# plumer/pbrs

Hardware: AMD Instinct MI355X
Metric: Msamples/s (higher is better)
Workload: dtype f32

## Files before the change

### pbrs_amd/csrc/device/scene.h

```cpp
#pragma once
#include <stddef.h>
#include <stdint.h>

#include "../../../include/pbrs_gpu.h"

constexpr uint32_t kBlock = 256;
constexpr size_t kLdsBytesPerCU = 160 * 1024;

struct pbrs_wnode;
struct DevScene {
    const pbrs_node* nodes;
    const pbrs_instance* inst;
    const pbrs_shape* shapes;
    const pbrs_mesh* meshes;
    const pbrs_tri_verts* tv;
    const pbrs_tri_shade* ts;
    const pbrs_material* mats;
    const pbrs_bxdf* bxdfs;
    const pbrs_area_light* alights;
    const pbrs_delta_light* dlights;
    uint32_t n_area, n_delta;
    float env[3];
    uint32_t has_env;
    uint32_t fast_slab;
    uint32_t exact_extent;
    uint32_t flat_off, n_flat;
    uint32_t features;
    uint32_t refill_below;
    uint32_t refill_below_shadow;
    const pbrs_texture* textures;
    const float* tex_floats;
    const uint32_t* tex_words;
    uint32_t env_kind, env_texture;
    float env_scale[3];
    const pbrs_fourier_table* fourier;
    uint32_t n_classes;
    const pbrs_wnode* wnodes;
    uint32_t wide_cap;
    uint32_t lds_off_words, lds_nodes, lds_tris, lds_inst, lds_shapes;
    const pbrs_node* nodes_top;
    uint32_t n_inst, n_shapes, n_tris, n_mats, n_bxdfs;
};

#define PBRS_INSTANCE_TRANSLATION 0x100u
#define PBRS_FEAT_ANALYTIC 1u
#define PBRS_FEAT_SHADING_CHECK 2u
#define PBRS_FEAT_FLAT_TLAS 4u
#define PBRS_FEAT_ALL 7u
#define PBRS_FEAT_EXTENT 256u
#define PBRS_FEAT_LONG_WALKS 8u
#define PBRS_FEAT_WIDE 16u
#define PBRS_FEAT_LDS_TOP 128u
#define PBRS_FEAT_LDS_SCENE 64u
#define PBRS_FEAT_FULL_STEPS 32u
#define PBRS_FLAT_TLAS_MIN 2u
#ifndef PBRS_FLAT_TLAS_MAX
#define PBRS_FLAT_TLAS_MAX 20u
#endif
#ifndef PBRS_FLAT_TLAS_MAX_ANYHIT
#define PBRS_FLAT_TLAS_MAX_ANYHIT 32u
#endif

struct pbrs_wnode {
    float lo[3][4];
    float hi[3][4];
    uint32_t child[4];
    uint32_t pad[4];
};
#ifndef PBRS_WIDE_STACK_MAX
#define PBRS_WIDE_STACK_MAX 16
#endif
#ifndef PBRS_WIDE_MIN_LEVELS
#define PBRS_WIDE_MIN_LEVELS 4u
#endif
#define PBRS_WREF_LEAF 0x80000000u
#define PBRS_WREF_NONE 0xffffffffu
#define PBRS_WREF_INDEX 0x07ffffffu
#define PBRS_WREF_AXIS_SHIFT 27
#define PBRS_WIDE_UNUSED_PLANE 1152921504606846976.0f

#ifndef PBRS_REFILL_BELOW_SHORT
#define PBRS_REFILL_BELOW_SHORT 20u
#endif
#ifndef PBRS_REFILL_BELOW_LONG
#define PBRS_REFILL_BELOW_LONG 48u
#endif
#ifndef PBRS_REFILL_BELOW_LONG_SHADOW
#define PBRS_REFILL_BELOW_LONG_SHADOW 40u
#endif
#define PBRS_LONG_WALK_HEIGHT 12u

#define PBRS_SHADE_LAMBERT 1u
#define PBRS_SHADE_LIGHT_SPHERE 2u
#define PBRS_SHADE_LIGHT_TRIANGLE 4u
#define PBRS_SHADE_FOURIER 8u
#define PBRS_SHADE_FOURIER_ONLY 16u
#define PBRS_SHADE_LDS_RECORDS 32u
#define PBRS_SHADE_LDS_TRIS 64u
#define PBRS_MAX_CLASSES 16u

#define PBRS_PERSISTENT_BLOCKS 1536
#ifndef PBRS_WORK_HEADS
#define PBRS_WORK_HEADS 8u
#endif
#define PBRS_WORK_HEAD_STRIDE 32u
#define PBRS_SORT_TILE 16384u
#define PBRS_QSPLIT_ON 1u
#define PBRS_QSPLIT_ENV 2u
```

### pbrs_amd/csrc/device/shadow.h

```cpp
#pragma once
#include "extend.h"

template <bool STATS, uint32_t FEAT>
__global__ void __launch_bounds__(256, STATS ? 3 : (FEAT & PBRS_FEAT_WIDE) ? PBRS_WIDE_SHADOW_WAVES : PBRS_SHADOW_WAVES)
    k_shadow(DevScene G, PathState st, const uint32_t* count, uint32_t* next, GlobalCounters* gc, const uint32_t* indirect, uint32_t* slow_list,
             uint32_t* slow_count) {
    extern __shared__ __attribute__((aligned(16))) uint32_t lds_stack[];
    const DevScene S = (!STATS && (FEAT & PBRS_FEAT_LDS_SCENE)) ? stage_scene(G, lds_stack) : (!STATS && (FEAT & PBRS_FEAT_LDS_TOP)) ? stage_top(G, lds_stack) : G;
    constexpr uint32_t ARITY = PBRS_WALK_ARITY(STATS, FEAT);
    constexpr bool WIDE = ARITY != 0u;
    const uint32_t n = indirect ? count[0] : count[1];
    LaneStack stk{lds_stack + threadIdx.x, st.sr[0], st.sr[1], 0u};
    Cnt<STATS> cnt;
    cnt.init();
    uint32_t nrays = 0;
    typename AnySel<ARITY, STATS, (FEAT & (PBRS_FEAT_ALL | PBRS_FEAT_LDS_TOP))>::type walk;
    walk.mode = PBRS_WALK_IDLE;
    PBRS_KP_DECL(walk);
    PBRS_TT_DECL;
    uint32_t item = 0, rec = 0;
    f3 l_vis = gray(0.0f);
    WaveWork work = wave_work_init(n);
    for (;;) {
        uint64_t live = __ballot(walk.mode == PBRS_WALK_NODE || walk.mode == PBRS_WALK_LEAF || walk.mode == PBRS_WALK_XFER);
        if ((uint32_t)__popcll(live) < S.refill_below_shadow) {
            PBRS_KP_WAVE(1);
            if constexpr (WIDE) {
                wave_append_slow(walk.mode == PBRS_WALK_SLOW, rec, slow_list, slow_count);
                if (walk.mode == PBRS_WALK_SLOW) walk.mode = PBRS_WALK_IDLE;
            }
            if (walk.mode == PBRS_WALK_DONE) {
                const bool occluded = walk.occluded;
                const uint32_t slot = item & PBRS_SLOT_MASK, r = item >> 31;
                if (item & 0x40000000u) {
                    if (!occluded) {
                        float* l = reinterpret_cast<float*>(st.L + slot);
                        l[0] = l_vis.x;
                        l[1] = l_vis.y;
                        l[2] = l_vis.z;
                    }
                } else {
                    at(st.occ[r], slot) = occluded ? 1 : 0;
                }
                walk.mode = PBRS_WALK_IDLE;
            }
            if (work.left()) {
                uint32_t idx = wave_fetch(work, walk.mode == PBRS_WALK_IDLE, next, n);
                if (idx != 0xffffffffu) {
                    if (indirect) idx = indirect[idx];
                    rec = idx;
                    stk.item = idx;
                    const float4 q0 = st.sr[0][idx], q1 = st.sr[1][idx];
                    item = __float_as_uint(q1.w);
                    if (item & 0x40000000u) l_vis = xyz(st.sr[2][idx]);
                    walk.start(S, mk3(q0.x, q0.y, q0.z), mk3(q1.x, q1.y, q1.z), q0.w, stk);
                    nrays++;
                    PBRS_KP_LANE(2, true);
                }
                if constexpr (WIDE) walk.scan_wave(S, stk);
                else walk.scan_wave(S, cnt);
                live = __ballot(walk.mode == PBRS_WALK_NODE || walk.mode == PBRS_WALK_LEAF || walk.mode == PBRS_WALK_XFER);
            }
            if (live == 0) {
                if constexpr (WIDE) {
                    walk.forget_reciprocals();
                    if (__ballot(walk.mode == PBRS_WALK_SLOW || walk.mode == PBRS_WALK_DONE)) continue;
                }
                break;
            }
        }
        PBRS_TT(0);
        PBRS_STEP_WALK(walk, S, stk, cnt, PBRS_SHD_XFER_MIN, PBRS_SHD_LEAF_MIN, PBRS_WALK_NSTEPS(FEAT, ARITY), ((FEAT & PBRS_FEAT_FULL_STEPS) != 0u));
        if constexpr (WIDE) walk.forget_reciprocals();
    }
    flush_counters<STATS>(cnt, gc, true, nrays, 0u);
    if (!STATS) PBRS_KP_FLUSH(1, walk);
    if (!STATS) PBRS_TT_FLUSH(1);
}
```

### pbrs_amd/csrc/device/traverse.h

```cpp
#pragma once
#include "shapes.h"

#include "probes.h"

struct RaySpace {
    f3 o, d;
    f3 nr;
    bool fast;
};
PD uint32_t dir_in_range(float x) {
    uint32_t e = (pn_bits(x) >> 23) & 0xffu;
    return (e - (127u - 40u) <= 80u) ? 1u : 0u;
}
PD uint32_t origin_in_range(float x) {
    uint32_t u = pn_bits(x) & 0x7fffffffu;
    uint32_t e = u >> 23;
    return ((u == 0u) | (e - (127u - 60u) <= 100u)) ? 1u : 0u;
}
PD RaySpace make_space(f3 o, f3 d, bool scene_ok) {
    RaySpace r;
    r.o = o;
    r.d = d;
    r.fast = ((scene_ok ? 1u : 0u) & dir_in_range(d.x) & dir_in_range(d.y) & dir_in_range(d.z) & origin_in_range(o.x) &
              origin_in_range(o.y) & origin_in_range(o.z)) != 0u;
// ... 695 lines not shown
            if (space == PBRS_SPACE_TRANSLATED) inst_kind |= 0x100u;
            stk.put(sp++, H.blas_root);
        } else if (inst_kind == PBRS_SHAPE_TRIANGLE) {
            leaf_a = H.blas_root;
            leaf_end = H.blas_root + 1u;
            mode = PBRS_WALK_LEAF;
        }
    }
    template <class AfterLeaf>
    PD void share_leaf(const DevScene& S, Cnt<STATS>& cnt, AfterLeaf after_leaf) {
        const bool tri_leaf = mode == PBRS_WALK_LEAF;
        TriShare sh;
        sh.build(tri_leaf ? leaf_end - leaf_a : 0u);
        if (sh.has[0] == 0) return;
        const f3 ho = sh.from_owner(C.o), hd = sh.from_owner(C.d);
        const float htmax = sh.from_owner(t_max);
        const uint32_t hti = sh.from_owner(leaf_a) + sh.k();
        bool hit = false;
        if (sh.helper()) {
            PBRS_TP(5);
            pbrs_tri_verts tv = load_tri(S.tv + hti);
            hit = mesh_tri_pred(tv, ho, hd, htmax);
        }
        const uint64_t hits = __ballot(hit);
        if (tri_leaf) {
            uint32_t tested = sh.cnt;
            bool occ = false;
#pragma unroll
            for (uint32_t j = 4u; j-- > 0u;) {
                if (j < sh.cnt && ((hits >> sh.pos(j)) & 1ull)) {
                    tested = j + 1u;
                    occ = true;
                }
            }
            if (STATS) cnt.c.triangles += tested;
            leaf_a += sh.cnt;
            mode = leaf_a != leaf_end ? PBRS_WALK_LEAF : after_leaf();
            if (occ) {
                occluded = true;
                mode = PBRS_WALK_DONE;
            }
        }
    }
    PD void leaf_wave(const DevScene& S, Cnt<STATS>& cnt) {
        share_leaf(S, cnt, [&]() __attribute__((always_inline)) { return sp == blas_base ? PBRS_WALK_XFER : PBRS_WALK_NODE; });
    }
    PD void analytic_visit(const DevScene& S, const pbrs_instance& in, Cnt<STATS>& cnt) {
        bool hit;
        {
            if (!(FEAT & PBRS_FEAT_ANALYTIC)) return;
            const f3 o = xf_apply(in.inv, C.o, 1.0f), d = xf_apply(in.inv, C.d, 0.0f);
            const float* p = S.shapes[in.shape_index].p;
            switch (inst_kind) {
                case PBRS_SHAPE_SPHERE:
                    CNT(spheres);
                    hit = sphere_occludes(ld3(p), p[3], o, d, t_max);
                    break;
                case PBRS_SHAPE_QUAD:
                    CNT(quads);
                    hit = quad_occludes(ld3(p), ld3(p + 3), ld3(p + 6), o, d, t_max);
                    break;
                case PBRS_SHAPE_CUBOID:
                    CNT(cuboids);
                    hit = slab_test(ld3(p), ld3(p + 3), o, d, t_max);
                    break;
                case PBRS_SHAPE_DISK:
                    CNT(disks);
                    hit = disk_occludes(ld3(p), ld3(p + 3), ld3(p + 6), o, d);
                    break;
                default:
                    hit = false;
                    break;
            }
        }
        if (hit) {
            occluded = true;
            mode = PBRS_WALK_DONE;
        }
    }
};

#define PBRS_WALK_SLOW 6u
#define PBRS_LEAF_UNVERIFIED 0xffffffffu
template <uint32_t FEAT>
struct AnyWalkW : AnyWalk<false, FEAT> {
    using B = AnyWalk<false, FEAT>;
    using B::C; using B::t_max; using B::leaf_a; using B::leaf_end; using B::inst_kind; using B::sp; using B::blas_base; using B::cand; using B::in_blas;
    using B::occluded; using B::moved; using B::mode;
    WideRay W;
    uint32_t cur;
    PD RaySpace exact_w() const {
        RaySpace E = C;
        E.nr = -W.r32;
        return E;
    }

    PD void start(const DevScene& S, f3 o, f3 d, float tmax, LaneStack stk) {
        B::start(S, o, d, tmax, stk);
        cur = PBRS_WREF_NONE;
        W.set(C);
        if (mode != PBRS_WALK_SCAN) mode = PBRS_WALK_SLOW;
    }
    PD void scan_wave(const DevScene& S, LaneStack) {
        Cnt<false> cnt;
        B::scan_wave(S, cnt);
    }
    PD uint32_t after_leaf() const { return sp == 0 ? B::exit_mode() : PBRS_WALK_NODE; }
    PD void hold_leaf(uint32_t ref) {
        leaf_a = ref & PBRS_WREF_INDEX;
        leaf_end = PBRS_LEAF_UNVERIFIED;
        mode = PBRS_WALK_LEAF;
    }
    PD void forget_reciprocals() { C.nr = gray(0.0f); }
    PD void node_step_fast(const DevScene& S, LaneStack stk, Cnt<false>& cnt) {
        if (cur == PBRS_WREF_NONE && sp == 0) return;
        node_step(S, stk, cnt);
    }
    PD void node_step(const DevScene& S, LaneStack stk, Cnt<false>&) {
        PBRS_TP(0);
        uint32_t e = cur;
        if (e == PBRS_WREF_NONE) {
            if (!in_blas) {
                if (cand == 0u) {
                    mode = PBRS_WALK_DONE;
                    return;
                }
                leaf_a = (uint32_t)__builtin_ctz(cand);
                cand &= cand - 1u;
                mode = PBRS_WALK_XFER;
                return;
            }
            if (sp == 0) {
                mode = B::exit_mode();
                return;
            }
            e = stk.get(--sp);
        }
        cur = PBRS_WREF_NONE;
        if (e & PBRS_WREF_LEAF) {
            hold_leaf(e);
            return;
        }
        PBRS_TP(1);
        const WideTest t = wide_test(S.wnodes, e, C, W, t_max);
        if (t.pass == 0u) {
            PBRS_TP(2);
            if (sp == 0) mode = B::exit_mode();
            return;
        }
        if (sp + 3 > (int)S.wide_cap) {
            mode = PBRS_WALK_SLOW;
            return;
        }
        const uint32_t first = wide_push(wide_order_any(t, C.d), stk, sp);
        if (first & PBRS_WREF_LEAF) hold_leaf(first);
        else cur = first;
    }
    PD void xfer_step(const DevScene& S, LaneStack stk, Cnt<false>& cnt) {
        if (in_blas) {
            const bool rebuilt = moved && !(inst_kind & 0x100u);
            mode = PBRS_WALK_NODE;
            in_blas = false;
            leave_instance(S, stk, !moved ? PBRS_SPACE_WORLD : (inst_kind & 0x100u) ? PBRS_SPACE_TRANSLATED : PBRS_SPACE_MOVED, C);
            if (rebuilt) W.set(C);
            return;
        }
        mode = PBRS_WALK_NODE;
        PBRS_TP(6);
        const pbrs_node leaf = load_node(S.nodes + S.flat_off + leaf_a);
        leaf_a = leaf.a;
        inst_kind = (leaf.b >> PBRS_TLAS_LEAF_KIND_SHIFT) & 7u;
        const pbrs_instance& in = S.inst[leaf_a];
        if ((FEAT & PBRS_FEAT_ANALYTIC) && inst_kind != PBRS_SHAPE_MESH && inst_kind != PBRS_SHAPE_TRIANGLE) {
            B::analytic_visit(S, in, cnt);
            return;
        }
        const InstHead H = load_inst_head(in);
        const uint32_t space = enter_instance(S, in, H.flags, C, inst_kind == PBRS_SHAPE_MESH, stk);
        moved = space != PBRS_SPACE_WORLD;
        in_blas = true;
        blas_base = 0;
        if (inst_kind == PBRS_SHAPE_MESH) {
            if (!C.fast) {
                mode = PBRS_WALK_SLOW;
                return;
            }
            if (space == PBRS_SPACE_TRANSLATED) inst_kind |= 0x100u;
            if (space == PBRS_SPACE_MOVED) W.set(C);
            const uint32_t wroot = H.wide_root;
            if (wroot == PBRS_WREF_NONE) {
                hold_leaf(H.blas_root);
                return;
            }
            if (!slab_rs(load_node(S.nodes + H.blas_root), exact_w(), t_max)) {
                mode = B::exit_mode();
                return;
            }
            cur = wroot;
        } else if (inst_kind == PBRS_SHAPE_TRIANGLE) {
            leaf_a = H.blas_root;
            leaf_end = H.blas_root + 1u;
            mode = PBRS_WALK_LEAF;
        }
    }
    PD void leaf_wave(const DevScene& S, Cnt<false>& cnt) {
        if (mode == PBRS_WALK_LEAF && leaf_end == PBRS_LEAF_UNVERIFIED) {
            PBRS_TP(3);
            const pbrs_node node = load_node(S.nodes + leaf_a);
            leaf_a = node.a;
            leaf_end = slab_rs(node, exact_w(), t_max) ? node.a + (node.b & ~PBRS_LEAF_FLAG) : node.a;
            if (leaf_end != leaf_a) PBRS_TP(4);
            if (leaf_end == leaf_a) mode = after_leaf();
        }
        B::share_leaf(S, cnt, [&]() __attribute__((always_inline)) { return after_leaf(); });
    }
};

template <bool STATS, uint32_t EXTRA = 0u>
PD void tlas_closest(const DevScene& S, bool active, f3 o, f3 d, float t_max, LaneStack stk, Hit& best, Cnt<STATS>& cnt) {
    ClosestWalk<STATS, PBRS_FEAT_ALL | EXTRA> w;
    w.start(S, o, d, t_max, stk);
    if (!active) w.mode = PBRS_WALK_DONE;
    w.scan_wave(S, cnt);
    while (__ballot(w.mode != PBRS_WALK_DONE)) {
        if (w.mode == PBRS_WALK_XFER) w.xfer_step(S, stk, cnt);
        if (w.mode == PBRS_WALK_NODE) w.node_step(S, stk, cnt);
        if (__ballot(w.mode == PBRS_WALK_LEAF)) w.leaf_wave(S, cnt);
    }
    w.finish(cnt);
    best = w.best;
}
template <bool STATS>
PD bool tlas_any(const DevScene& S, bool active, f3 o, f3 d, float t_max, LaneStack stk, Cnt<STATS>& cnt) {
    AnyWalk<STATS, PBRS_FEAT_ALL> w;
    w.start(S, o, d, t_max, stk);
    if (!active) w.mode = PBRS_WALK_DONE;
    w.scan_wave(S, cnt);
    while (__ballot(w.mode != PBRS_WALK_DONE)) {
        if (w.mode == PBRS_WALK_XFER) w.xfer_step(S, stk, cnt);
        if (w.mode == PBRS_WALK_NODE) w.node_step(S, stk, cnt);
        if (__ballot(w.mode == PBRS_WALK_LEAF)) w.leaf_wave(S, cnt);
    }
    return w.occluded;
}
PD bool tlas_any_wide(const DevScene& S, bool active, f3 o, f3 d, float t_max, LaneStack stk, bool& slow) {
    Cnt<false> cnt;
    AnyWalkW<PBRS_FEAT_ALL> w;
    w.start(S, o, d, t_max, stk);
    if (!active) w.mode = PBRS_WALK_DONE;
    w.scan_wave(S, stk);
    while (__ballot(w.mode == PBRS_WALK_NODE || w.mode == PBRS_WALK_LEAF || w.mode == PBRS_WALK_XFER)) {
        if (w.mode == PBRS_WALK_XFER) w.xfer_step(S, stk, cnt);
        if (w.mode == PBRS_WALK_NODE) w.node_step(S, stk, cnt);
        if (__ballot(w.mode == PBRS_WALK_LEAF)) w.leaf_wave(S, cnt);
    }
    slow = w.mode == PBRS_WALK_SLOW;
    bool occ = w.occluded;
    if (__ballot(slow)) {
        const bool o2 = tlas_any<false>(S, active && slow, o, d, t_max, stk, cnt);
        if (slow) occ = o2;
    }
    return occ;
}
```

### pbrs_amd/csrc/device/wide.h

```cpp
#pragma once
#include "scene.h"
#include "shapes.h"


struct WideRay {
    f3 r32;
    uint32_t nb;
    PD void set(const RaySpace& C) {
        r32 = -C.nr;
        nb = (C.d.x > 0.0f ? 0u : 48u) | (C.d.y > 0.0f ? 16u : 64u) << 8 | (C.d.z > 0.0f ? 32u : 80u) << 16;
    }
    PD uint32_t nx() const { return nb & 0xffu; }
    PD uint32_t ny() const { return (nb >> 8) & 0xffu; }
    PD uint32_t nz() const { return nb >> 16; }
};

struct WideTest {
    uint32_t pass;
    uint32_t child[4];
    PD int axis_x() const { return (int)((child[0] >> PBRS_WREF_AXIS_SHIFT) & 3u); }
    PD int axis_left() const { return (int)((child[0] >> (PBRS_WREF_AXIS_SHIFT + 2)) & 3u); }
    PD int axis_right() const { return (int)((child[2] >> PBRS_WREF_AXIS_SHIFT) & 3u); }
};
PD WideTest wide_test(const pbrs_wnode* nodes, uint32_t wi, const RaySpace& C, const WideRay& W, float t_max) {
    const char* base = reinterpret_cast<const char*>(nodes);
    const uint32_t at = wi * (uint32_t)sizeof(pbrs_wnode);
    const float4 nx = *reinterpret_cast<const float4*>(base + (at + W.nx())), ny = *reinterpret_cast<const float4*>(base + (at + W.ny())),
                 nz = *reinterpret_cast<const float4*>(base + (at + W.nz()));
    const float4 fx = *reinterpret_cast<const float4*>(base + (at + (48u - W.nx()))), fy = *reinterpret_cast<const float4*>(base + (at + (80u - W.ny()))),
                 fz = *reinterpret_cast<const float4*>(base + (at + (112u - W.nz())));
    const uint4 ch = *reinterpret_cast<const uint4*>(base + (at + 96u));
    WideTest t;
    t.child[0] = ch.x, t.child[1] = ch.y, t.child[2] = ch.z, t.child[3] = ch.w;
    const uint32_t p0 = pn_slab_filter(nx.x, ny.x, nz.x, fx.x, fy.x, fz.x, C.o.x, C.o.y, C.o.z, W.r32.x, W.r32.y, W.r32.z, t_max) ? 1u : 0u;
    const uint32_t p1 = pn_slab_filter(nx.y, ny.y, nz.y, fx.y, fy.y, fz.y, C.o.x, C.o.y, C.o.z, W.r32.x, W.r32.y, W.r32.z, t_max) ? 2u : 0u;
    const uint32_t p2 = pn_slab_filter(nx.z, ny.z, nz.z, fx.z, fy.z, fz.z, C.o.x, C.o.y, C.o.z, W.r32.x, W.r32.y, W.r32.z, t_max) ? 4u : 0u;
    const uint32_t p3 = pn_slab_filter(nx.w, ny.w, nz.w, fx.w, fy.w, fz.w, C.o.x, C.o.y, C.o.z, W.r32.x, W.r32.y, W.r32.z, t_max) ? 8u : 0u;
    t.pass = p0 | p1 | p2 | p3;
    asm volatile("" : "+v"(t.child[0]), "+v"(t.child[1]), "+v"(t.child[2]), "+v"(t.child[3]));
    return t;
}

struct WideOrder {
    uint32_t r[4], p[4];
};
PD WideOrder wide_order_any(const WideTest& t, f3 d) {
    const bool sx = !(comp(d, t.axis_x()) > 0.0f);
    const uint32_t q0 = t.pass & 1u, q1 = (t.pass >> 1) & 1u, q2 = (t.pass >> 2) & 1u, q3 = (t.pass >> 3) & 1u;
    WideOrder o;
    o.r[0] = sx ? t.child[3] : t.child[0], o.r[1] = sx ? t.child[2] : t.child[1], o.r[2] = sx ? t.child[1] : t.child[2], o.r[3] = sx ? t.child[0] : t.child[3];
    o.p[0] = sx ? q3 : q0, o.p[1] = sx ? q2 : q1, o.p[2] = sx ? q1 : q2, o.p[3] = sx ? q0 : q3;
    return o;
}
PD uint32_t wide_push(const WideOrder& o, LaneStack stk, int& sp) {
    const uint32_t any01 = o.p[0] | o.p[1], any012 = any01 | o.p[2];
    if (o.p[3] & any012) stk.put(sp, o.r[3]);
    if (o.p[2] & any01) stk.put(sp + (int)o.p[3], o.r[2]);
    if (o.p[1] & o.p[0]) stk.put(sp + (int)(o.p[3] + o.p[2]), o.r[1]);
    sp += (int)(o.p[0] + o.p[1] + o.p[2] + o.p[3]) - 1;
    return o.p[0] ? o.r[0] : o.p[1] ? o.r[1] : o.p[2] ? o.r[2] : o.r[3];
}
```

### pbrs_amd/csrc/host/scene_prepare.cpp

```cpp
#include "scene_prepare.h"

#include <algorithm>
#include <cstring>
#include <map>
#include <string>

#include "../../../include/pbrs_numeric.h"
#include "../../../include/pbrs_scene_spec.h"
#include "../device/split_planes.h"

namespace pbrs {
namespace {

SceneCheck refuse(int code, const char* message) { return SceneCheck{code, message, SceneLevels{}}; }

void tree_heights(const pbrs_node* nodes, uint32_t n, std::vector<uint32_t>& h) {
    h.assign(n, 1u);
    for (uint32_t i = n; i-- > 0;)
        if (!(nodes[i].b & PBRS_LEAF_FLAG)) h[i] = std::max(h[i + 1], h[nodes[i].a]) + 1u;
}

SceneLevels scene_levels(const pbrs_scene_desc& d) {
    SceneLevels l;
    std::vector<uint32_t> th, bh;
// ... 177 lines not shown
    PreparedScene P;
    DevScene& S = P.S;
    SceneFacts& f = P.facts;
    P.stack_depth = lv.stack;
    {
        bool ok = true;
        for (uint32_t i = 0; i < d.n_tlas_nodes && ok; ++i)
            for (int a = 0; a < 3; ++a) ok = ok && coord_ok(d.tlas_nodes[i].min[a]) && coord_ok(d.tlas_nodes[i].max[a]);
        for (uint32_t i = 0; i < d.n_blas_nodes && ok; ++i)
            for (int a = 0; a < 3; ++a) ok = ok && coord_ok(d.blas_nodes[i].min[a]) && coord_ok(d.blas_nodes[i].max[a]);
        S.fast_slab = ok ? 1u : 0u;
    }
    S.exact_extent = lv.exact_extent ? 1u : 0u;

    const bool scan = tlas_scanned(d);
    std::vector<pbrs_node>& nodes = P.nodes;
    nodes.assign(d.tlas_nodes, d.tlas_nodes + d.n_tlas_nodes);
    S.flat_off = (uint32_t)nodes.size();
    if (scan)
        for (uint32_t i = 0; i < d.n_tlas_nodes; ++i)
            if (d.tlas_nodes[i].b & PBRS_LEAF_FLAG) nodes.push_back(d.tlas_nodes[i]);
    S.n_flat = (uint32_t)nodes.size() - S.flat_off;
    const uint64_t blas_off = nodes.size();
    nodes.insert(nodes.end(), d.blas_nodes, d.blas_nodes + d.n_blas_nodes);
    for (size_t i = blas_off; i < nodes.size(); ++i)
        if (!(nodes[i].b & PBRS_LEAF_FLAG)) nodes[i].a += (uint32_t)blas_off;
    P.node_planes.assign(nodes.size(), 0u);
    if (S.fast_slab != 0u)
        for (size_t i = blas_off; i < nodes.size(); ++i)
            if (!(nodes[i].b & PBRS_LEAF_FLAG)) P.node_planes[i] = split_planes(nodes, (uint32_t)i);
    P.walk_bytes = nodes.size() * sizeof(pbrs_node) + (uint64_t)d.n_triangles * sizeof(pbrs_tri_verts) + (uint64_t)d.n_instances * sizeof(pbrs_instance);

    std::vector<pbrs_instance>& inst = P.inst;
    inst.assign(d.instances, d.instances + d.n_instances);
    std::vector<uint32_t> mat_class(d.n_materials, 0u);
    {
        std::vector<std::string> sigs;
        for (uint32_t m = 0; m < d.n_materials; ++m) {
            const pbrs_material& mt = d.materials[m];
            if (mt.n_bxdfs == 0) continue;
            std::string sig;
            for (uint32_t k = 0; k < mt.n_bxdfs; ++k) {
                const pbrs_bxdf& bx = d.bxdfs[mt.first_bxdf + k];
                sig += (char)('a' + bx.kind);
                sig += (char)('a' + (bx.kind == PBRS_BXDF_SPECULAR ? bx.intrusion : 0u));
                sig += (char)('a' + (bx.kind == PBRS_BXDF_DIFFUSE ? bx.oren_nayar : bx.fresnel));
                sig += (char)('a' + (bx.kind == PBRS_BXDF_MICROFACET && bx.alpha_x != bx.alpha_y ? 1 : 0));
                sig += bx.tex ? 't' : '-';
            }
            size_t at = 0;
            while (at < sigs.size() && sigs[at] != sig) ++at;
            if (at == sigs.size()) sigs.push_back(sig);
            mat_class[m] = (uint32_t)std::min<size_t>(at + 1, PBRS_MAX_CLASSES - 1);
        }
        S.n_classes = (uint32_t)std::min<size_t>(sigs.size(), PBRS_MAX_CLASSES - 1);
        const std::string lam_sig = {(char)('a' + PBRS_BXDF_DIFFUSE), 'a', 'a', 'a', '-'};
        for (size_t at = 0; at < sigs.size() && at + 1 < PBRS_MAX_CLASSES - 1; ++at)
            if (sigs[at] == lam_sig) f.lambert_class = (uint32_t)at + 1;
        const std::string fou_sig = {(char)('a' + PBRS_BXDF_FOURIER), 'a', 'a', 'a', '-'};
        for (size_t at = 0; at < sigs.size() && at + 1 < PBRS_MAX_CLASSES - 1; ++at)
            if (sigs[at] == fou_sig) f.fourier_class = (uint32_t)at + 1;
    }
    for (pbrs_instance& in : inst) {
        in.pad[0] = mat_class[in.material];
        if (in.shape_kind == PBRS_SHAPE_MESH) in.blas_root += (uint32_t)blas_off;
        bool linear_identity = true;
        for (int r = 0; r < 3; ++r)
            for (int k = 0; k < 3; ++k) linear_identity = linear_identity && pn_bits(in.inv[r][k]) == pn_bits(r == k ? 1.0f : 0.0f);
        in.flags &= ~PBRS_INSTANCE_TRANSLATION;
        if (linear_identity) in.flags |= PBRS_INSTANCE_TRANSLATION;
    }
    for (pbrs_instance& in : inst) in.pad[1] = PBRS_WREF_NONE;
    S.wide_cap = 4u;
    if (scan && S.fast_slab != 0u) {
        std::vector<pbrs_wnode>& wide = P.wide;
        std::map<uint32_t, uint32_t> wide_of_root;
        uint32_t levels = 0;
        for (pbrs_instance& in : inst) {
            if (in.shape_kind != PBRS_SHAPE_MESH || (nodes[in.blas_root].b & PBRS_LEAF_FLAG)) continue;
            auto it = wide_of_root.find(in.blas_root);
            if (it == wide_of_root.end()) it = wide_of_root.emplace(in.blas_root, build_wide(nodes, in.blas_root, wide, 0u, levels)).first;
            in.pad[1] = it->second;
        }
        if (levels >= PBRS_WIDE_MIN_LEVELS && wide.size() * sizeof(pbrs_wnode) < (1ull << 32)) {
            P.walk_bytes += wide.size() * sizeof(pbrs_wnode);
            S.wide_cap = std::max(4u, std::min(3u * levels + 1u, (uint32_t)PBRS_WIDE_STACK_MAX));
            P.wide_levels = levels;
        } else {
            wide.clear();
            for (pbrs_instance& in : inst) in.pad[1] = PBRS_WREF_NONE;
        }
    }

    S.n_area = d.n_area_lights;
    S.n_delta = d.n_delta_lights;
    S.env_kind = d.env_kind;
    S.env_texture = d.env_texture;
    std::memcpy(S.env_scale, d.env_scale, sizeof S.env_scale);
    std::memcpy(S.env, d.env_constant, sizeof S.env);
    S.has_env = (d.env_kind != PBRS_ENV_CONSTANT || !(S.env[0] <= 0.0f && S.env[1] <= 0.0f && S.env[2] <= 0.0f)) ? 1u : 0u;
    S.refill_below = lv.max_blas >= PBRS_LONG_WALK_HEIGHT ? PBRS_REFILL_BELOW_LONG : PBRS_REFILL_BELOW_SHORT;
    S.refill_below_shadow = lv.max_blas >= PBRS_LONG_WALK_HEIGHT ? PBRS_REFILL_BELOW_LONG_SHADOW : PBRS_REFILL_BELOW_SHORT;
    if (dev.refill_below) S.refill_below = S.refill_below_shadow = *dev.refill_below;
    f.long_walks = (S.n_flat ? 0u : lv.tlas) + lv.max_blas >= PBRS_LONG_WALK_HEIGHT;
    f.full_steps = S.fast_slab == 0u;
    f.tlas_scanned = S.n_flat != 0u;
    S.features = (S.n_flat != 0u && d.n_instances <= PBRS_FLAT_TLAS_MAX) ? PBRS_FEAT_FLAT_TLAS : 0u;
    f.wide_ok = S.fast_slab != 0u && P.wide_levels >= PBRS_WIDE_MIN_LEVELS;
    for (uint32_t i = 0; i < d.n_instances; ++i) {
        const pbrs_instance& in = d.instances[i];
        if (in.shape_kind == PBRS_SHAPE_MESH) {
            if (!(in.mesh_flags & PBRS_MESH_SHADING_OK_MASK)) S.features |= PBRS_FEAT_SHADING_CHECK;
        } else if (in.shape_kind != PBRS_SHAPE_TRIANGLE) {
            S.features |= PBRS_FEAT_ANALYTIC;
        }
    }
    f.features = S.features;
    f.exact_extent = lv.exact_extent;
    f.n_classes = S.n_classes;
    P.has_vis_records = d.n_materials > 0;
    for (uint32_t i = 0; i < d.n_materials; ++i) P.has_vis_records = P.has_vis_records && d.materials[i].vis_bxdf != 0;
    for (uint32_t i = 0; i < d.n_bxdfs; ++i) {
        f.textured = f.textured || (d.bxdfs[i].tex & ~PBRS_BXDF_TEX_DROP_IF_BLACK) != 0;
        f.fourier = f.fourier || d.bxdfs[i].kind == PBRS_BXDF_FOURIER;
    }
    f.lambert = !f.textured;
    for (uint32_t i = 0; i < d.n_materials && f.lambert; ++i) {
        const pbrs_material& m = d.materials[i];
        f.lambert = m.n_bxdfs <= 1;
        for (uint32_t k = 0; k < m.n_bxdfs && f.lambert; ++k) {
            const pbrs_bxdf& bx = d.bxdfs[m.first_bxdf + k];
            f.lambert = bx.kind == PBRS_BXDF_DIFFUSE && bx.oren_nayar == 0 && bx.tex == 0;
        }
    }
    if (d.n_area_lights) {
        const uint32_t k0 = d.area_lights[0].shape_kind;
        bool same = true;
        for (uint32_t i = 1; i < d.n_area_lights; ++i) same = same && d.area_lights[i].shape_kind == k0;
        if (same && k0 == PBRS_SHAPE_SPHERE) f.light_spec = PBRS_SHADE_LIGHT_SPHERE;
        if (same && k0 == PBRS_SHAPE_TRIANGLE) f.light_spec = PBRS_SHADE_LIGHT_TRIANGLE;
    }
    f.stack_bytes = (size_t)lv.stack * kBlock * sizeof(uint32_t);
    f.wide_stack_bytes = (size_t)S.wide_cap * kBlock * sizeof(uint32_t);
    f.scene_bytes = nodes.size() * sizeof(pbrs_node) + (size_t)d.n_triangles * sizeof(pbrs_tri_verts) + (size_t)d.n_instances * sizeof(pbrs_instance) +
                    (size_t)d.n_shapes * sizeof(pbrs_shape);
    f.top_bytes = (size_t)d.n_tlas_nodes * sizeof(pbrs_node);
    S.n_inst = d.n_instances; S.n_shapes = d.n_shapes; S.n_tris = d.n_triangles; S.n_mats = d.n_materials; S.n_bxdfs = d.n_bxdfs;
    f.shade_rec_bytes = (size_t)d.n_instances * sizeof(pbrs_instance) + (size_t)d.n_shapes * sizeof(pbrs_shape) + (size_t)d.n_materials * sizeof(pbrs_material) +
                        (size_t)d.n_bxdfs * sizeof(pbrs_bxdf) + (size_t)d.n_area_lights * sizeof(pbrs_area_light) + (size_t)d.n_delta_lights * sizeof(pbrs_delta_light);
    f.shade_tri_bytes = (size_t)d.n_triangles * (sizeof(pbrs_tri_verts) + sizeof(pbrs_tri_shade));
    const size_t budget = 16u << 10;
    f.shade_lds = f.shade_rec_bytes + f.shade_tri_bytes <= budget ? PBRS_SHADE_LDS_ALL : f.shade_rec_bytes <= budget ? PBRS_SHADE_LDS_RECORDS : 0u;
    return P;
}

}
```

### pbrs_amd/csrc/host/scene_prepare.h

```cpp
#pragma once
#include <cstdint>
#include <vector>

#include "../device/scene.h"
#include "kernel_choice.h"

namespace pbrs {

struct SceneLevels {
    uint32_t tlas = 0;
    uint32_t max_blas = 0;
    uint32_t stack = 0;
    bool exact_extent = false;
};
struct SceneCheck {
    int code = PBRS_OK;
    const char* message = nullptr;
    SceneLevels levels;
};
SceneCheck check_scene(const pbrs_scene_desc& d);

struct PreparedScene {
    DevScene S{};
    std::vector<pbrs_node> nodes;
    std::vector<uint32_t> node_planes;
    std::vector<pbrs_instance> inst;
    std::vector<pbrs_wnode> wide;
    uint32_t wide_levels = 0;
    SceneFacts facts;
    uint32_t stack_depth = 0;
    bool has_vis_records = false;
    uint64_t walk_bytes = 0;
};
PreparedScene prepare_scene(const pbrs_scene_desc& d, const SceneLevels& levels, const DevOverrides& dev);

}
```

### pbrs_amd/csrc/pbrs_gpu.hip

```cpp
#include <hip/hip_runtime.h>

#include <algorithm>
#include <cmath>
#include <cstdio>
#include <cstdlib>
#include <cstring>
#include <utility>
#include <mutex>
#include <optional>
#include <string>
#include <vector>

#include "../../include/pbrs_gpu.h"
#include "device/raygen.h"
#include "device/class_sort.h"
#include "device/accumulate.h"
#include "device/dev_kernels.h"
#include "kernel_tables.h"
#include "host/scene_prepare.h"
#include "host/arg_checks.h"
#include "host/pass_plan.h"
#include "device/aov.h"
#include "device/film.h"
#include "device/denoise.h"
// ... 112 lines not shown
        bool in_flight = false;
    } pass_set[2];
    int cur_set = 0;
    hipStream_t main_stream = nullptr;
    hipStream_t second_stream = nullptr;
    bool overlap_passes = true;
    uint32_t overlap_from = 2;
    size_t cap_pixels = 0;
    float* sum = nullptr;
    float* rgb_dev = nullptr;
    GlobalCounters* gcnt = nullptr;
    unsigned long long* nonfinite = nullptr;
    unsigned long long* bounce_acc = nullptr;

    std::vector<StageEvent> events;
    size_t events_used = 0;
    std::vector<hipEvent_t> total_ev;
    pbrs_stats pending{};
    bool pending_counters = false, pending_times = false;
    DevOverrides dev;
    KernelPlan plan;
    int split_decision = 0;
    unsigned long long* split_host = nullptr;
    hipEvent_t split_ev = nullptr;
    bool split_probe_in_flight = false;
    bool has_vis_records = false;
    uint64_t pending_closest = 0;
    pbrs_intersect_info last_intersect{};
    DeviceBuffer buf[N_BUFFERS];
};

namespace {

#define HIPCHK(ctx, expr)                                                                             \
    do {                                                                                              \
        hipError_t e_ = (expr);                                                                       \
        if (e_ != hipSuccess) {                                                                       \
            (ctx)->error = std::string(#expr) + ": " + hipGetErrorString(e_);                         \
            (void)hipGetLastError();  \
            return PBRS_E_DEVICE;                                                                     \
        }                                                                                             \
    } while (0)

struct CallAllocs {
    std::vector<void*> held;
    CallAllocs() = default;
    CallAllocs(const CallAllocs&) = delete;
    CallAllocs& operator=(const CallAllocs&) = delete;
    ~CallAllocs() {
        for (void* p : held) (void)hipFree(p);
    }
    template <class T>
    hipError_t alloc(T** p, size_t bytes) {
        void* q = nullptr;
        const hipError_t e = hipMalloc(&q, bytes);
        if (e == hipSuccess) held.push_back(q);
        *p = static_cast<T*>(q);
        return e;
    }
};

int fail(pbrs_ctx* c, int code, const char* msg) {
    c->error = msg;
    return code;
}
int fail(pbrs_ctx* c, const Refusal& r) { return r.code ? fail(c, r.code, r.message) : PBRS_OK; }

int enter(pbrs_ctx* c, const Refusal& r) {
    if (!c) return PBRS_E_INVALID;
    if (r.code) return fail(c, r);
    HIPCHK(c, hipSetDevice(c->device));
    return PBRS_OK;
}

template <class T>
int upload(pbrs_ctx* c, const T* src, size_t n, const T** dst) {
    *dst = nullptr;
    size_t bytes = (n ? n : 1) * sizeof(T);
    void* p = nullptr;
    HIPCHK(c, hipMalloc(&p, bytes));
    c->scene_allocs.push_back(p);
    if (n) HIPCHK(c, hipMemcpy(p, src, n * sizeof(T), hipMemcpyHostToDevice));
    *dst = static_cast<const T*>(p);
    return PBRS_OK;
}

void free_scene(pbrs_ctx* c) {
    for (void* p : c->scene_allocs) (void)hipFree(p);
    c->scene_allocs.clear();
    c->has_scene = false;
}

pbrs_ctx::PassSet& cur(pbrs_ctx* c) { return c->pass_set[c->cur_set]; }

void use_pass_set(pbrs_ctx* c, int k) {
    c->cur_set = k;
    c->stream = c->main_stream;
}

void free_paths(pbrs_ctx::PassSet& set) {
    set.cap_slots = 0;
    set.st = PathState{};
    set.neeq = nullptr;
    set.rng_hi0 = nullptr;
    set.slow = nullptr;
    if (set.state_mem) (void)hipFree(set.state_mem);
    set.state_mem = nullptr;
}

void free_work(pbrs_ctx* c) {
    for (pbrs_ctx::PassSet& set : c->pass_set) free_paths(set);
    c->cap_pixels = 0;
    if (c->sum) (void)hipFree(c->sum);
    if (c->rgb_dev) (void)hipFree(c->rgb_dev);
    c->sum = nullptr;
    c->rgb_dev = nullptr;
}

template <class T>
T* column(void* mem, const PathLayout& lay, uint32_t col) {
    return reinterpret_cast<T*>(static_cast<char*>(mem) + lay.offset[col]);
}
constexpr bool columns_hold(uint32_t first, uint32_t n, size_t elem) {
    for (uint32_t i = first; i < first + n; ++i)
        if (kPathColumns[i].elem != elem) return false;
    return true;
}
static_assert(columns_hold(COL_Q, 14, sizeof(float4)) && columns_hold(COL_OCC, 1, sizeof(uint8_t)) && columns_hold(COL_NEEQ, 2, sizeof(uint32_t)) &&
                  columns_hold(COL_CLS, 1, sizeof(uint8_t)) && columns_hold(COL_SLOW, 2, sizeof(uint32_t)) && columns_hold(COL_CLASS_RANGE, 1, sizeof(uint2)) &&
                  columns_hold(COL_RNG_HI0, 1, sizeof(uint32_t)),
              "kPathColumns and PathState disagree about a column's element");

int ensure_work(pbrs_ctx* c, pbrs_ctx::PassSet& set, size_t n_slots, size_t n_pixels) {
    if (n_slots > set.cap_slots) {
        free_paths(set);
        const PathLayout lay = path_layout(n_slots);
        void* mem = nullptr;
        hipError_t e = hipMalloc(&mem, lay.total);
        if (e != hipSuccess) {
            c->error = std::string("hipMalloc of the path state (") + std::to_string(lay.total >> 20) + " MiB): " + hipGetErrorString(e);
            (void)hipGetLastError();
            return PBRS_E_DEVICE;
        }
        set.state_mem = mem;
        PathState s{};
        for (uint32_t half = 0; half < 2; ++half)
            for (uint32_t k = 0; k < 3; ++k) s.q[half][k] = column<float4>(mem, lay, COL_Q + 3 * half + k);
        s.hit = column<float4>(mem, lay, COL_HIT);
        s.L = column<float4>(mem, lay, COL_L);
        for (uint32_t k = 0; k < 3; ++k) s.nee[k] = column<float4>(mem, lay, COL_NEE + k);
        for (uint32_t k = 0; k < 3; ++k) s.sr[k] = column<float4>(mem, lay, COL_SR + k);
        s.occ[0] = column<uint8_t>(mem, lay, COL_OCC);
        s.occ[1] = s.occ[0] + n_slots;
        set.neeq = column<uint32_t>(mem, lay, COL_NEEQ);
        s.perm = column<uint32_t>(mem, lay, COL_PERM);
        s.cls = column<uint8_t>(mem, lay, COL_CLS);
        set.slow = column<uint32_t>(mem, lay, COL_SLOW);
        s.tile_hist = column<uint32_t>(mem, lay, COL_TILE_HIST);
        s.class_range = column<uint2>(mem, lay, COL_CLASS_RANGE);
        set.rng_hi0 = column<uint32_t>(mem, lay, COL_RNG_HI0);
        set.st = s;
        set.cap_slots = n_slots;
    }
    if (n_pixels > c->cap_pixels) {
        c->cap_pixels = 0;
        if (c->sum) (void)hipFree(c->sum);
// ... 547 lines not shown
        hipEvent_t ev = nullptr;
        ok = hipEventCreate(&ev) == hipSuccess;
        if (ok) c->total_ev.push_back(ev);
    }
    for (pbrs_ctx::PassSet& set : c->pass_set) ok = ok && hipMalloc(reinterpret_cast<void**>(&set.counters), kCounters.words * sizeof(uint32_t)) == hipSuccess;
    ok = ok && hipMalloc(reinterpret_cast<void**>(&c->gcnt), 2 * sizeof(GlobalCounters)) == hipSuccess &&
         hipMalloc(reinterpret_cast<void**>(&c->nonfinite), sizeof(unsigned long long)) == hipSuccess &&
         hipMalloc(reinterpret_cast<void**>(&c->bounce_acc), (2 * PBRS_STATS_MAX_BOUNCES + 2) * sizeof(unsigned long long)) == hipSuccess &&
         hipMemset(c->bounce_acc, 0, (2 * PBRS_STATS_MAX_BOUNCES + 2) * sizeof(unsigned long long)) == hipSuccess &&
         hipMemset(c->nonfinite, 0, sizeof(unsigned long long)) == hipSuccess &&
         hipHostMalloc(reinterpret_cast<void**>(&c->split_host), 2 * sizeof(unsigned long long), hipHostMallocDefault) == hipSuccess &&
         hipEventCreateWithFlags(&c->split_ev, hipEventDisableTiming) == hipSuccess;
    ok = ok && configure_kernels(c) == PBRS_OK;
    if (!ok) {
        pbrs_destroy(c);
        return PBRS_E_DEVICE;
    }
    *out = c;
    return PBRS_OK;
}

void pbrs_destroy(pbrs_ctx* c) {
    if (!c) return;
    (void)hipSetDevice(c->device);
    if (c->stream) (void)hipStreamSynchronize(c->stream);
    if (c->second_stream) (void)hipStreamSynchronize(c->second_stream);
    free_scene(c);
    free_work(c);
    for (DeviceBuffer& b : c->buf)
        if (b.p) (void)hipFree(b.p);
    for (pbrs_ctx::PassSet& set : c->pass_set)
        if (set.counters) (void)hipFree(set.counters);
    for (int k = 0; k < 2; ++k)
        if (c->pass_set[k].accumulated) (void)hipEventDestroy(c->pass_set[k].accumulated);
    for (int k = 0; k < 2; ++k)
        if (c->pass_set[k].late) (void)hipEventDestroy(c->pass_set[k].late);
    if (c->second_stream) (void)hipStreamDestroy(c->second_stream);
    if (c->gcnt) (void)hipFree(c->gcnt);
    if (c->nonfinite) (void)hipFree(c->nonfinite);
    if (c->bounce_acc) (void)hipFree(c->bounce_acc);
    if (c->split_host) (void)hipHostFree(c->split_host);
    if (c->split_ev) (void)hipEventDestroy(c->split_ev);
    for (auto& e : c->events) {
        (void)hipEventDestroy(e.a);
        (void)hipEventDestroy(e.b);
    }
    for (auto& e : c->total_ev) (void)hipEventDestroy(e);
    if (c->own_stream) (void)hipStreamDestroy(c->own_stream);
    delete c;
}

const char* pbrs_last_error(const pbrs_ctx* c) { return c ? c->error.c_str() : "null context"; }

int pbrs_set_stream(pbrs_ctx* c, void* hip_stream) {
    if (!c) return PBRS_E_INVALID;
    c->main_stream = hip_stream ? static_cast<hipStream_t>(hip_stream) : c->own_stream;
    c->stream = c->main_stream;
    return PBRS_OK;
}

int pbrs_set_pass_overlap(pbrs_ctx* c, int enabled) {
    if (!c) return PBRS_E_INVALID;
    c->overlap_passes = enabled != 0;
    return PBRS_OK;
}

int pbrs_upload_scene(pbrs_ctx* c, const pbrs_scene_desc* d) {
    if (!c || !d) return PBRS_E_INVALID;
    HIPCHK(c, hipSetDevice(c->device));
    const SceneCheck chk = check_scene(*d);
    if (chk.code != PBRS_OK) return fail(c, chk.code, chk.message);
    PreparedScene P = prepare_scene(*d, chk.levels, c->dev);
    const KernelChoice choice = choose_kernels(P.facts, c->dev);
    KernelPlan plan;
    if (!bind_kernels(choice, plan)) return fail(c, PBRS_E_DEVICE, "no kernel instantiation for this scene's feature set");
    (void)hipStreamSynchronize(c->stream);
    (void)hipStreamSynchronize(c->second_stream);
    free_scene(c);
    c->plan = plan;
    DevScene S = P.S;
    int rc;
    for (size_t i = 0; i < P.nodes.size(); ++i) P.nodes[i].b |= P.node_planes[i];
    if ((rc = upload(c, P.nodes.data(), P.nodes.size(), &S.nodes))) return rc;
    if (!P.wide.empty() && (rc = upload(c, P.wide.data(), P.wide.size(), &S.wnodes))) return rc;
    if ((rc = upload(c, P.inst.data(), P.inst.size(), &S.inst))) return rc;
    if ((rc = upload(c, d->shapes, d->n_shapes, &S.shapes))) return rc;
    if ((rc = upload(c, d->meshes, d->n_meshes, &S.meshes))) return rc;
    if ((rc = upload(c, d->tri_verts, d->n_triangles, &S.tv))) return rc;
    if ((rc = upload(c, d->tri_shade, d->n_triangles, &S.ts))) return rc;
    if ((rc = upload(c, d->materials, d->n_materials, &S.mats))) return rc;
    if ((rc = upload(c, d->bxdfs, d->n_bxdfs, &S.bxdfs))) return rc;
    if ((rc = upload(c, d->area_lights, d->n_area_lights, &S.alights))) return rc;
    if ((rc = upload(c, d->delta_lights, d->n_delta_lights, &S.dlights))) return rc;
    if ((rc = upload(c, d->textures, d->n_textures, &S.textures))) return rc;
    if ((rc = upload(c, d->tex_floats, d->n_tex_floats, &S.tex_floats))) return rc;
    if ((rc = upload(c, d->tex_words, d->n_tex_words, &S.tex_words))) return rc;
    if ((rc = upload(c, d->fourier_tables, d->n_fourier_tables, &S.fourier))) return rc;
    const bool lds_scene = choice.lds_staging == PBRS_FEAT_LDS_SCENE;
    S.lds_off_words = P.stack_depth * kBlock;
    S.lds_nodes = lds_scene ? (uint32_t)P.nodes.size() : choice.lds_staging == PBRS_FEAT_LDS_TOP ? d->n_tlas_nodes : 0u;
    S.lds_tris = lds_scene ? d->n_triangles : 0u;
    S.lds_inst = lds_scene ? d->n_instances : 0u;
    S.lds_shapes = lds_scene ? d->n_shapes : 0u;
    c->S = S;
    c->overlap_from = c->dev.overlap_from.value_or(P.walk_bytes <= (4ull << 20) ? 2u : 4u);
    c->has_vis_records = P.has_vis_records;
    c->stack_depth = P.stack_depth;
    c->has_scene = true;
    c->split_decision = 0;
    c->split_probe_in_flight = false;
    return PBRS_OK;
}

int pbrs_render_tile_passes_device(pbrs_ctx* c, const pbrs_camera* cam, const pbrs_render_params* p, float* rgb_out_device,
                                   const pbrs_aov_buffers* aovs_device, float* variance_device, const pbrs_matte_params* params,
                                   const pbrs_matte_buffers* matte_device, const pbrs_pass_buffers* passes_device, pbrs_stats* stats_out) {
    if (!c) return PBRS_E_INVALID;
    if (!rgb_out_device) return fail(c, PBRS_E_INVALID, "null output");
    return render(c, cam, p, nullptr, make_targets(rgb_out_device, aovs_device, variance_device, params, matte_device, passes_device), false, stats_out);
}

int pbrs_render_tile_matte_device(pbrs_ctx* c, const pbrs_camera* cam, const pbrs_render_params* p, float* rgb_out_device,
                                  const pbrs_aov_buffers* aovs_device, float* variance_device, const pbrs_matte_params* params,
                                  const pbrs_matte_buffers* matte_device, pbrs_stats* stats_out) {
    return pbrs_render_tile_passes_device(c, cam, p, rgb_out_device, aovs_device, variance_device, params, matte_device, nullptr, stats_out);
}

int pbrs_render_tile_aovs_var_device(pbrs_ctx* c, const pbrs_camera* cam, const pbrs_render_params* p, float* rgb_out_device,
                                     const pbrs_aov_buffers* aovs_device, float* variance_device, pbrs_stats* stats_out) {
    return pbrs_render_tile_matte_device(c, cam, p, rgb_out_device, aovs_device, variance_device, nullptr, nullptr, stats_out);
}

int pbrs_render_tile_aovs_device(pbrs_ctx* c, const pbrs_camera* cam, const pbrs_render_params* p, float* rgb_out_device, const pbrs_aov_buffers* aovs_device,
                                 pbrs_stats* stats_out) {
    return pbrs_render_tile_matte_device(c, cam, p, rgb_out_device, aovs_device, nullptr, nullptr, nullptr, stats_out);
}

int pbrs_render_tile_device(pbrs_ctx* c, const pbrs_camera* cam, const pbrs_render_params* p, float* rgb_out_device, pbrs_stats* stats_out) {
    return pbrs_render_tile_matte_device(c, cam, p, rgb_out_device, nullptr, nullptr, nullptr, nullptr, stats_out);
}

int pbrs_render_tile_passes(pbrs_ctx* c, const pbrs_camera* cam, const pbrs_render_params* p, float* rgb_out_host, const pbrs_aov_buffers* aovs_host,
                            float* variance_host, const pbrs_matte_params* params, const pbrs_matte_buffers* matte_host, const pbrs_pass_buffers* passes_host,
                            pbrs_stats* stats_out) {
    if (!c) return PBRS_E_INVALID;
    if (!rgb_out_host) return fail(c, PBRS_E_INVALID, "null output");
    return render(c, cam, p, nullptr, make_targets(rgb_out_host, aovs_host, variance_host, params, matte_host, passes_host), true, stats_out);
}

int pbrs_render_tile_matte(pbrs_ctx* c, const pbrs_camera* cam, const pbrs_render_params* p, float* rgb_out_host, const pbrs_aov_buffers* aovs_host,
                           float* variance_host, const pbrs_matte_params* params, const pbrs_matte_buffers* matte_host, pbrs_stats* stats_out) {
    return pbrs_render_tile_passes(c, cam, p, rgb_out_host, aovs_host, variance_host, params, matte_host, nullptr, stats_out);
}

int pbrs_render_tile_aovs_var(pbrs_ctx* c, const pbrs_camera* cam, const pbrs_render_params* p, float* rgb_out_host, const pbrs_aov_buffers* aovs_host,
                              float* variance_host, pbrs_stats* stats_out) {
    return pbrs_render_tile_matte(c, cam, p, rgb_out_host, aovs_host, variance_host, nullptr, nullptr, stats_out);
}

int pbrs_render_tile_aovs(pbrs_ctx* c, const pbrs_camera* cam, const pbrs_render_params* p, float* rgb_out_host, const pbrs_aov_buffers* aovs_host,
                          pbrs_stats* stats_out) {
    return pbrs_render_tile_matte(c, cam, p, rgb_out_host, aovs_host, nullptr, nullptr, nullptr, stats_out);
}

int pbrs_render_tile(pbrs_ctx* c, const pbrs_camera* cam, const pbrs_render_params* p, float* rgb_out_host, pbrs_stats* stats_out) {
    return pbrs_render_tile_matte(c, cam, p, rgb_out_host, nullptr, nullptr, nullptr, nullptr, stats_out);
}
// ... 699 lines not shown
```

Baseline: 1684.

## Pack small wide-BVH leaf triangle ranges into child refs and verify lazily

Wide-BVH leaf references with up to four triangles now hold the first triangle index and count directly. Any-hit traversal can then test triangles without first fetching the leaf's binary node to check its exact slab. The slab check is deferred until a shadow ray is found occluded; it uses a triangle-to-leaf table appended after the wide nodes, and reverts the occlusion if the box test fails. This trades a node load on every packed leaf for extra triangle tests, a settle pass in the shadow loop, and a larger device allocation.

Result: faster. 1706 (median of 6 runs) (+1.3%).

```diff
diff --git a/pbrs_amd/csrc/device/scene.h b/pbrs_amd/csrc/device/scene.h
--- a/pbrs_amd/csrc/device/scene.h
+++ b/pbrs_amd/csrc/device/scene.h
@@ -40,6 +40,7 @@
     uint32_t lds_off_words, lds_nodes, lds_tris, lds_inst, lds_shapes;
     const pbrs_node* nodes_top;
     uint32_t n_inst, n_shapes, n_tris, n_mats, n_bxdfs;
+    uint32_t n_wnodes;
 };
 
 #define PBRS_INSTANCE_TRANSLATION 0x100u
@@ -77,6 +78,18 @@
 #define PBRS_WREF_NONE 0xffffffffu
 #define PBRS_WREF_INDEX 0x07ffffffu
 #define PBRS_WREF_AXIS_SHIFT 27
+#define PBRS_WREF_PACKED 0x04000000u
+#define PBRS_WREF_TRI_BITS 24
+#define PBRS_WREF_TRI 0x00ffffffu
+#define PBRS_WREF_COUNT_SHIFT 24
+#define PBRS_WREF_COUNT_MAX 4u
+static_assert((PBRS_WREF_PACKED & PBRS_WREF_INDEX) == PBRS_WREF_PACKED && PBRS_WREF_PACKED < (1u << PBRS_WREF_AXIS_SHIFT), "the packed flag lies inside the index bits, below the axes");
+static_assert(PBRS_WREF_TRI == (1u << PBRS_WREF_TRI_BITS) - 1u && PBRS_WREF_COUNT_SHIFT == PBRS_WREF_TRI_BITS, "first triangle: the low bits, the count above them");
+static_assert(((PBRS_WREF_COUNT_MAX - 1u) << PBRS_WREF_COUNT_SHIFT) < PBRS_WREF_PACKED && (PBRS_WREF_PACKED >> PBRS_WREF_COUNT_SHIFT) == PBRS_WREF_COUNT_MAX,
+              "two bits of count - 1 between the triangle index and the flag");
+static_assert((PBRS_WREF_PACKED | ((PBRS_WREF_COUNT_MAX - 1u) << PBRS_WREF_COUNT_SHIFT) | PBRS_WREF_TRI) == PBRS_WREF_INDEX, "flag, count and triangle fill the 27 bits exactly");
+static_assert(PBRS_WREF_TRI_BITS >= 24, "a mesh of 2^24 triangles (indices 0 .. 2^24 - 1) packs");
+static_assert((PBRS_WREF_LEAF | PBRS_WREF_INDEX | (15u << PBRS_WREF_AXIS_SHIFT)) == 0xffffffffu && PBRS_WREF_LEAF == (1u << 31), "leaf bit, four axis bits, 27 index bits");
 #define PBRS_WIDE_UNUSED_PLANE 1152921504606846976.0f
 
 #ifndef PBRS_REFILL_BELOW_SHORT
diff --git a/pbrs_amd/csrc/device/shadow.h b/pbrs_amd/csrc/device/shadow.h
--- a/pbrs_amd/csrc/device/shadow.h
+++ b/pbrs_amd/csrc/device/shadow.h
@@ -28,6 +28,8 @@
             if constexpr (WIDE) {
                 wave_append_slow(walk.mode == PBRS_WALK_SLOW, rec, slow_list, slow_count);
                 if (walk.mode == PBRS_WALK_SLOW) walk.mode = PBRS_WALK_IDLE;
+                walk.settle(S);
+                live = __ballot(walk.mode == PBRS_WALK_NODE || walk.mode == PBRS_WALK_LEAF || walk.mode == PBRS_WALK_XFER);
             }
             if (walk.mode == PBRS_WALK_DONE) {
                 const bool occluded = walk.occluded;
diff --git a/pbrs_amd/csrc/device/traverse.h b/pbrs_amd/csrc/device/traverse.h
--- a/pbrs_amd/csrc/device/traverse.h
+++ b/pbrs_amd/csrc/device/traverse.h
@@ -801,6 +801,7 @@
 
 #define PBRS_WALK_SLOW 6u
 #define PBRS_LEAF_UNVERIFIED 0xffffffffu
+#define PBRS_KIND_BOX_OWED 0x200u
 template <uint32_t FEAT>
 struct AnyWalkW : AnyWalk<false, FEAT> {
     using B = AnyWalk<false, FEAT>;
@@ -826,9 +827,17 @@
     }
     PD uint32_t after_leaf() const { return sp == 0 ? B::exit_mode() : PBRS_WALK_NODE; }
     PD void hold_leaf(uint32_t ref) {
-        leaf_a = ref & PBRS_WREF_INDEX;
-        leaf_end = PBRS_LEAF_UNVERIFIED;
+        const bool packed = (ref & PBRS_WREF_PACKED) != 0u;
+        leaf_a = ref & (packed ? PBRS_WREF_TRI : PBRS_WREF_INDEX);
+        leaf_end = packed ? leaf_a + ((ref >> PBRS_WREF_COUNT_SHIFT) & (PBRS_WREF_COUNT_MAX - 1u)) + 1u : PBRS_LEAF_UNVERIFIED;
+        inst_kind = packed ? inst_kind | PBRS_KIND_BOX_OWED : inst_kind & ~PBRS_KIND_BOX_OWED;
+        if (packed) PBRS_TP(3);
         mode = PBRS_WALK_LEAF;
+    }
+    PD bool verify_leaf(const DevScene& S, uint32_t tri) {
+        const bool pass = slab_rs(load_node(S.nodes + tri_leaf(S, tri)), exact_w(), t_max);
+        if (pass) PBRS_TP(4);
+        return pass;
     }
     PD void forget_reciprocals() { C.nr = gray(0.0f); }
     PD void node_step_fast(const DevScene& S, LaneStack stk, Cnt<false>& cnt) {
@@ -933,6 +942,15 @@
         }
         B::share_leaf(S, cnt, [&]() __attribute__((always_inline)) { return after_leaf(); });
     }
+    PD void settle(const DevScene& S) {
+        if (mode == PBRS_WALK_DONE && occluded && (inst_kind & PBRS_KIND_BOX_OWED)) {
+            inst_kind &= ~PBRS_KIND_BOX_OWED;
+            if (!verify_leaf(S, leaf_a - 1u)) {
+                occluded = false;
+                mode = after_leaf();
+            }
+        }
+    }
 };
 
 template <bool STATS, uint32_t EXTRA = 0u>
@@ -968,11 +986,14 @@
     w.start(S, o, d, t_max, stk);
     if (!active) w.mode = PBRS_WALK_DONE;
     w.scan_wave(S, stk);
-    while (__ballot(w.mode == PBRS_WALK_NODE || w.mode == PBRS_WALK_LEAF || w.mode == PBRS_WALK_XFER)) {
-        if (w.mode == PBRS_WALK_XFER) w.xfer_step(S, stk, cnt);
-        if (w.mode == PBRS_WALK_NODE) w.node_step(S, stk, cnt);
-        if (__ballot(w.mode == PBRS_WALK_LEAF)) w.leaf_wave(S, cnt);
-    }
+    do {
+        while (__ballot(w.mode == PBRS_WALK_NODE || w.mode == PBRS_WALK_LEAF || w.mode == PBRS_WALK_XFER)) {
+            if (w.mode == PBRS_WALK_XFER) w.xfer_step(S, stk, cnt);
+            if (w.mode == PBRS_WALK_NODE) w.node_step(S, stk, cnt);
+            if (__ballot(w.mode == PBRS_WALK_LEAF)) w.leaf_wave(S, cnt);
+        }
+        w.settle(S);
+    } while (__ballot(w.mode == PBRS_WALK_NODE || w.mode == PBRS_WALK_LEAF || w.mode == PBRS_WALK_XFER));
     slow = w.mode == PBRS_WALK_SLOW;
     bool occ = w.occluded;
     if (__ballot(slow)) {
diff --git a/pbrs_amd/csrc/device/wide.h b/pbrs_amd/csrc/device/wide.h
--- a/pbrs_amd/csrc/device/wide.h
+++ b/pbrs_amd/csrc/device/wide.h
@@ -2,6 +2,8 @@
 #include "scene.h"
 #include "shapes.h"
 
+
+PD uint32_t tri_leaf(const DevScene& S, uint32_t t) { return reinterpret_cast<const uint32_t*>(S.wnodes + S.n_wnodes)[t]; }
 
 struct WideRay {
     f3 r32;
diff --git a/pbrs_amd/csrc/host/scene_prepare.cpp b/pbrs_amd/csrc/host/scene_prepare.cpp
--- a/pbrs_amd/csrc/host/scene_prepare.cpp
+++ b/pbrs_amd/csrc/host/scene_prepare.cpp
@@ -283,8 +283,14 @@
             if (it == wide_of_root.end()) it = wide_of_root.emplace(in.blas_root, build_wide(nodes, in.blas_root, wide, 0u, levels)).first;
             in.pad[1] = it->second;
         }
-        if (levels >= PBRS_WIDE_MIN_LEVELS && wide.size() * sizeof(pbrs_wnode) < (1ull << 32)) {
+        if (levels >= PBRS_WIDE_MIN_LEVELS && wide.size() * sizeof(pbrs_wnode) < (1ull << 32) && nodes.size() <= PBRS_WREF_PACKED) {
             P.walk_bytes += wide.size() * sizeof(pbrs_wnode);
+            P.tri_leaf.assign(d.n_triangles, 0xffffffffu);
+            for (size_t i = blas_off; i < nodes.size(); ++i)
+                if (nodes[i].b & PBRS_LEAF_FLAG)
+                    for (uint32_t t = nodes[i].a, end = t + (nodes[i].b & ~PBRS_LEAF_FLAG); t < end; ++t) P.tri_leaf[t] = (uint32_t)i;
+            P.walk_bytes += P.tri_leaf.size() * sizeof(uint32_t);
+            S.n_wnodes = (uint32_t)wide.size();
             S.wide_cap = std::max(4u, std::min(3u * levels + 1u, (uint32_t)PBRS_WIDE_STACK_MAX));
             P.wide_levels = levels;
         } else {
@@ -355,4 +361,23 @@
     return P;
 }
 
-}
+uint32_t pack_wide_leaves(PreparedScene& P) {
+    uint32_t packed = 0;
+    for (pbrs_wnode& w : P.wide)
+        for (uint32_t k = 0; k < 4; ++k) {
+            const uint32_t ref = w.child[k];
+            if (ref == PBRS_WREF_NONE || !(ref & PBRS_WREF_LEAF)) continue;
+            const uint32_t ni = ref & PBRS_WREF_INDEX;
+            const pbrs_node& n = P.nodes[ni];
+            const uint32_t cnt = n.b & ~PBRS_LEAF_FLAG;
+            if (cnt == 0u || cnt > PBRS_WREF_COUNT_MAX || n.a > PBRS_WREF_TRI) continue;
+            bool own = true;
+            for (uint32_t j = 0; j < cnt; ++j) own = own && P.tri_leaf[n.a + j] == ni;
+            if (!own) continue;
+            w.child[k] = (ref & ~PBRS_WREF_INDEX) | PBRS_WREF_PACKED | (cnt - 1u) << PBRS_WREF_COUNT_SHIFT | n.a;
+            ++packed;
+        }
+    return packed;
+}
+
+}
diff --git a/pbrs_amd/csrc/host/scene_prepare.h b/pbrs_amd/csrc/host/scene_prepare.h
--- a/pbrs_amd/csrc/host/scene_prepare.h
+++ b/pbrs_amd/csrc/host/scene_prepare.h
@@ -26,6 +26,7 @@
     std::vector<uint32_t> node_planes;
     std::vector<pbrs_instance> inst;
     std::vector<pbrs_wnode> wide;
+    std::vector<uint32_t> tri_leaf;
     uint32_t wide_levels = 0;
     SceneFacts facts;
     uint32_t stack_depth = 0;
@@ -33,5 +34,6 @@
     uint64_t walk_bytes = 0;
 };
 PreparedScene prepare_scene(const pbrs_scene_desc& d, const SceneLevels& levels, const DevOverrides& dev);
+uint32_t pack_wide_leaves(PreparedScene& P);
 
 }
diff --git a/pbrs_amd/csrc/pbrs_gpu.hip b/pbrs_amd/csrc/pbrs_gpu.hip
--- a/pbrs_amd/csrc/pbrs_gpu.hip
+++ b/pbrs_amd/csrc/pbrs_gpu.hip
@@ -218,6 +218,18 @@
     c->scene_allocs.push_back(p);
     if (n) HIPCHK(c, hipMemcpy(p, src, n * sizeof(T), hipMemcpyHostToDevice));
     *dst = static_cast<const T*>(p);
+    return PBRS_OK;
+}
+
+int upload_wide(pbrs_ctx* c, const PreparedScene& P, const pbrs_wnode** dst) {
+    *dst = nullptr;
+    const size_t wide_bytes = P.wide.size() * sizeof(pbrs_wnode), table_bytes = P.tri_leaf.size() * sizeof(uint32_t);
+    void* p = nullptr;
+    HIPCHK(c, hipMalloc(&p, wide_bytes + table_bytes));
+    c->scene_allocs.push_back(p);
+    HIPCHK(c, hipMemcpy(p, P.wide.data(), wide_bytes, hipMemcpyHostToDevice));
+    if (table_bytes) HIPCHK(c, hipMemcpy(static_cast<char*>(p) + wide_bytes, P.tri_leaf.data(), table_bytes, hipMemcpyHostToDevice));
+    *dst = static_cast<const pbrs_wnode*>(p);
     return PBRS_OK;
 }
 
@@ -931,7 +943,8 @@
     int rc;
     for (size_t i = 0; i < P.nodes.size(); ++i) P.nodes[i].b |= P.node_planes[i];
     if ((rc = upload(c, P.nodes.data(), P.nodes.size(), &S.nodes))) return rc;
-    if (!P.wide.empty() && (rc = upload(c, P.wide.data(), P.wide.size(), &S.wnodes))) return rc;
+    pack_wide_leaves(P);
+    if (!P.wide.empty() && (rc = upload_wide(c, P, &S.wnodes))) return rc;
     if ((rc = upload(c, P.inst.data(), P.inst.size(), &S.inst))) return rc;
     if ((rc = upload(c, d->shapes, d->n_shapes, &S.shapes))) return rc;
     if ((rc = upload(c, d->meshes, d->n_meshes, &S.meshes))) return rc;
```
